# apchenstu/mvsnerf

Hardware: AMD Instinct MI355X
Metric: rendered rays/sec (1024-ray batch, 128 samples) (higher is better)
Workload: dtype f32; 1 GPU; config 2: 3 source views 512x640, 128 depth planes, pad 24 (volume 128x176x208x8), 1024 rays x 128 samples per step, MLP arithmetic fp32, render-only (volume pre-built); weights=mvsnerf-v0 checkpoint, volume=mvsnet-encode, parallelism=ray-sharded x1, no data-path collective

## Files before the change

mvsnerf_amd/csrc/mlp.hip:

```cpp
#include "common.h"
#include "mlp_layout.h"
#include "lds_dma.h"
#include "knobs.h"

using namespace mlp;
typedef float f32x2 __attribute__((ext_vector_type(2)));

struct PackArgs {
    const float* w[11];
    const float* b[11];
    int F;
};

__device__ inline void pack_segment(float* __restrict__ dst, const float* __restrict__ W, int ld, int col_off,
                                    int kmap, int steps, int nb, int F, int tid, int nthreads)
{
    const int total = steps * nb * 64;
    for (int i = tid; i < total; i += nthreads) {
        const int j = i & 3;
        const int lane = (i >> 2) & 63;
        const int rest = i >> 8;
        const int b = rest % nb, t = (rest / nb) * 4 + j;
        const int col = kmap_col(kmap, t, lane >> 5, F);
        const int row = b * 32 + (lane & 31);
        dst[i] = col < 0 ? 0.0f : W[(size_t)row * ld + col_off + col];
    }
}

__global__ __launch_bounds__(256) void mlp_pack_kernel(PackArgs a, float* __restrict__ packed)
{
    const Layout L = layout(a.F);
    const int tid = blockIdx.x * blockDim.x + threadIdx.x, nt = gridDim.x * blockDim.x;
    pack_segment(packed + L.biasw, a.w[6], a.F, 0, K_FEAT, L.fsteps, 4, a.F, tid, nt);
    pack_segment(packed + L.l0, a.w[0], PE_DIM, 0, K_PE, PE_STEPS, 4, a.F, tid, nt);
    pack_segment(packed + L.l1, a.w[1], WIDTH, 0, K_ACT, ACT_STEPS, 4, a.F, tid, nt);
    pack_segment(packed + L.l2, a.w[2], WIDTH, 0, K_ACT, ACT_STEPS, 4, a.F, tid, nt);
// ... 122 lines not shown
    const float v = (q & 1) ? cs : sn;
    return (q & 2) ? -v : v;
}

__device__ __forceinline__ float pe_operand(int t, int half, float px, float py, float pz)
{
    if (t == 0) return half ? py : px;
    if (t == 1) return half ? 0.0f : pz;
    const int j = t - 2, f = j / 3, c = j - 3 * f;
    const float x = (c == 0 ? px : c == 1 ? py : pz) * (float)(1 << f);
    return pe_sin_or_cos(x, half);
}


constexpr int SLAB_FLOATS = 8704;
constexpr int PIPE_LDS_FLOATS = 2 * SLAB_FLOATS + V_TOTAL;

__device__ __forceinline__ void slab_dma(float* __restrict__ dst, const float* __restrict__ src, int n_floats, int wave, int lane)
{
    lds_dma<4>(dst, src, n_floats >> 8, wave, lane);
}
template <int N_FLOATS>
__device__ __forceinline__ void slab_dma_c(float* __restrict__ dst, const float* __restrict__ src, int wave, int lane)
{
    lds_dma_c<4, N_FLOATS / 256>(dst, src, wave, lane);
}

__device__ __forceinline__ void slab_sync()
{
    asm volatile("s_waitcnt vmcnt(0)" ::: "memory");
    __syncthreads();
}

template <bool ALPHA_ONLY, bool SAVE>
__device__ __forceinline__ void mlp_fwd_pipe_tile(
    const unsigned tile, const float* __restrict__ packed, int F, const float* __restrict__ ndc, int ndc_stride,
    const float* __restrict__ feat, int feat_stride, const float* __restrict__ dirs, int dirs_stride,
    int64_t P, int S, float* __restrict__ raw, float* __restrict__ saved, long long* __restrict__ census)
{
    extern __shared__ __attribute__((aligned(16))) float lds[];
    long long t_start = 0, c_start = 0;
    if (census) { t_start = wall_clock64(); c_start = __builtin_amdgcn_s_memtime(); }
    int stamp_i = 4;
    auto stamp = [&]() { if (census && threadIdx.x == 0 && stamp_i < 16) census[tile * 16 + stamp_i] = wall_clock64(); ++stamp_i; };
    float* buf0 = lds;
    float* buf1 = lds + SLAB_FLOATS;
    float* vec = lds + 2 * SLAB_FLOATS;
    constexpr int G = 1;
    const Layout L = layout(F);
    const int tid = threadIdx.x, lane = tid & 63;
    const int wave = __builtin_amdgcn_readfirstlane(tid >> 6);
    const int half = lane >> 5;
    const int64_t p_raw = ((int64_t)tile * 4 + wave) * 32 + (lane & 31);
    const bool live = p_raw < P;
    const int64_t p = live ? p_raw : P - 1;
    float* sv = nullptr;
    if (SAVE) sv = saved + ((int64_t)tile * 4 + wave) * (SLOTS_SAVED * 64) + lane;
    auto save = [&](int slot, float v) { if (SAVE) sv[slot * 64] = v; };
    constexpr int HALF = (int)(ACT_STEPS / 2) * 4 * 64;

    slab_dma(buf0, packed + L.biasw, (int)seg_floats(L.fsteps, 4), wave, lane);
    slab_dma_c<(int)seg_floats(PE_STEPS, 4)>(buf1, packed + L.l0, wave, lane);
    for (int i = tid; i < V_TOTAL; i += 256) vec[i] = packed[L.vec + i];
    const float px = ndc[p * ndc_stride + 0], py = ndc[p * ndc_stride + 1], pz = ndc[p * ndc_stride + 2];
    float fv[MAX_F / 2];
    {
        const float* fp = feat + p * feat_stride + half * (F / 2);
#pragma unroll
        for (int i = 0; i < MAX_F / 2; ++i) fv[i] = i < F / 2 ? fp[i] : 0.0f;
    }
    float bias[64], h[64];
    auto pe = [&](int g, int t) { return pe_operand(t, half, px, py, pz); };
    auto hlo = [&](int g, int t) { return h[t]; };
    auto hhi = [&](int g, int t) { return h[32 + t]; };

    slab_sync();
    stamp();
    {
        f32x16 acc[G][4];
        init_acc<4, G>(acc, vec + V_BIASG + half * 64);
        auto fb = [&](int g, int t) { return fv[t]; };
        switch (L.fsteps) {
            case 4:  gemm_stage<1, 4, G>(buf0, acc, lane, fb); break;
            case 8:  gemm_stage<2, 4, G>(buf0, acc, lane, fb); break;
            case 12: gemm_stage<3, 4, G>(buf0, acc, lane, fb); break;
            case 16: gemm_stage<4, 4, G>(buf0, acc, lane, fb); break;
            default: gemm_stage<5, 4, G>(buf0, acc, lane, fb); break;
        }
#pragma unroll
        for (int q = 0; q < 64; ++q) { bias[q] = acc[0][q >> 4][q & 15]; save(S_BM + q, bias[q]); }
        if (SAVE) {
#pragma unroll
            for (int t = 0; t < 16; ++t) save(S_FV + t, fv[t]);
#pragma unroll
            for (int t = 0; t < PE_STEPS; ++t) save(S_E + t, pe_operand(t, half, px, py, pz));
        }
    }
    stamp();
    slab_sync();
    slab_dma_c<HALF>(buf0, packed + L.l1, wave, lane);
    {
        f32x16 acc[G][4];
        init_acc<4, G>(acc, vec + V_L0 + half * 64);
        gemm_stage<PE_STEPS / 4, 4, G>(buf1, acc, lane, pe);
#pragma unroll
        for (int q = 0; q < 64; q += 2) {
            const f32x2 m2 = f32x2{acc[0][q >> 4][q & 15], acc[0][q >> 4][(q & 15) + 1]} * f32x2{bias[q], bias[q + 1]};
            h[q] = fmaxf(m2[0], 0.0f); h[q + 1] = fmaxf(m2[1], 0.0f);
            save(S_H + q, h[q]); save(S_H + q + 1, h[q + 1]);
// ... 15 lines not shown
            h[q] = fmaxf(m2[0], 0.0f); h[q + 1] = fmaxf(m2[1], 0.0f);
            save(S_H + layer * 64 + q, h[q]); save(S_H + layer * 64 + q + 1, h[q + 1]);
        }
        stamp();
    }
    float sigma;
    {
        f32x16 acc[G][4];
        slab_sync();
        init_acc<4, G>(acc, vec + V_L0 + 128 * 5 + half * 64);
        gemm_stage<PE_STEPS / 4, 4, G>(buf0, acc, lane, pe, [&]() { slab_dma_c<HALF>(buf1, packed + L.l5b, wave, lane); });
        slab_sync();
        gemm_stage<8, 4, G>(buf1, acc, lane, hlo, [&]() { slab_dma_c<HALF>(buf0, packed + L.l5b + HALF, wave, lane); });
        slab_sync();
        gemm_stage<8, 4, G>(buf0, acc, lane, hhi, [&]() { if (!ALPHA_ONLY) slab_dma_c<HALF>(buf1, packed + L.feat, wave, lane); });
#pragma unroll
        for (int q = 0; q < 64; q += 2) {
            const f32x2 m2 = f32x2{acc[0][q >> 4][q & 15], acc[0][q >> 4][(q & 15) + 1]} * f32x2{bias[q], bias[q + 1]};
            h[q] = fmaxf(m2[0], 0.0f); h[q + 1] = fmaxf(m2[1], 0.0f);
            save(S_H + 5 * 64 + q, h[q]); save(S_H + 5 * 64 + q + 1, h[q + 1]);
        }
        const float* wa = vec + V_WA + half * 64;
        float part = 0.0f;
#pragma unroll
        for (int q = 0; q < 64; ++q) part = fmaf(wa[q], h[q], part);
        part += __shfl_xor(part, 32);
        sigma = fmaxf(part + vec[V_BA], 0.0f);
    }
    stamp();
    if (ALPHA_ONLY) {
        if (live && half == 0) raw[p_raw] = sigma;
        return;
    }
    {
        f32x16 acc[G][4];
        slab_sync();
        init_acc<4, G>(acc, vec + V_FEAT + half * 64);
        gemm_stage<8, 4, G>(buf1, acc, lane, hlo, [&]() { slab_dma_c<HALF>(buf0, packed + L.feat + HALF, wave, lane); });
        slab_sync();
        gemm_stage<8, 4, G>(buf0, acc, lane, hhi, [&]() { slab_dma_c<(int)seg_floats(VIEW_STEPS, 2)>(buf1, packed + L.views, wave, lane); });
#pragma unroll
        for (int q = 0; q < 64; ++q) { h[q] = acc[0][q >> 4][q & 15]; save(S_FE + q, h[q]); }
    }
    stamp();
    {
        float d0, d1, d2;
        { const int64_t ray = p / S; d0 = dirs[ray * dirs_stride + 0]; d1 = dirs[ray * dirs_stride + 1]; d2 = dirs[ray * dirs_stride + 2]; }
        f32x16 acc[G][2];
        slab_sync();
        init_acc<2, G>(acc, vec + V_VIEWS + half * 32);
        gemm_stage<VIEW_STEPS / 4, 2, G>(buf1, acc, lane, [&](int g, int t) {
            return t < ACT_STEPS ? h[t < ACT_STEPS ? t : 0] : t == ACT_STEPS ? (half ? d1 : d0) : t == ACT_STEPS + 1 ? (half ? 0.0f : d2) : 0.0f;
        });
        if (SAVE) {
#pragma unroll
            for (int q = 0; q < 32; ++q) save(S_HV + q, fmaxf(acc[0][q >> 4][q & 15], 0.0f));
            save(S_DR + 0, half ? d1 : d0);
            save(S_DR + 1, half ? 0.0f : d2);
        }
        float rgb[3];
#pragma unroll
        for (int c = 0; c < 3; ++c) {
            const float* wr = vec + V_WR + c * 64 + half * 32;
            float part = 0.0f;
#pragma unroll
            for (int q = 0; q < 32; ++q) part = fmaf(wr[q], fmaxf(acc[0][q >> 4][q & 15], 0.0f), part);
            part += __shfl_xor(part, 32);
            const float x = part + vec[V_BR + c];
            rgb[c] = 1.0f / (1.0f + expf(-x));
        }
        if (live && half == 0) *reinterpret_cast<f32x4*>(raw + p_raw * 4) = f32x4{rgb[0], rgb[1], rgb[2], sigma};
    }
    if (census && tid == 0) {
        census[tile * 16 + 0] = t_start;
        census[tile * 16 + 1] = wall_clock64();
        census[tile * 16 + 2] = __builtin_amdgcn_s_getreg((4) | (0 << 6) | (31 << 11));
        census[tile * 16 + 3] = __builtin_amdgcn_s_getreg((20) | (0 << 6) | (31 << 11));
        census[tile * 16 + 13] = __builtin_amdgcn_s_memtime() - c_start;
    }
}

template <bool ALPHA_ONLY, bool SAVE>
__global__ __launch_bounds__(256, 2) void mlp_fwd_pipe_kernel(
    const float* __restrict__ packed, int F, const float* __restrict__ ndc, int ndc_stride,
    const float* __restrict__ feat, int feat_stride, const float* __restrict__ dirs, int dirs_stride,
    int64_t P, int S, float* __restrict__ raw, float* __restrict__ saved, long long* __restrict__ census)
{
    mlp_fwd_pipe_tile<ALPHA_ONLY, SAVE>(blockIdx.x, packed, F, ndc, ndc_stride, feat, feat_stride, dirs, dirs_stride, P, S, raw, saved, census);
}

template <bool ALPHA_ONLY>
__global__ __launch_bounds__(256, 2) void mlp_fwd_pipe_if_kernel(
    const float* __restrict__ packed, int F, const float* __restrict__ ndc, int ndc_stride,
    const float* __restrict__ feat, int feat_stride, const float* __restrict__ dirs, int dirs_stride,
    int64_t P, int S, float* __restrict__ raw, const int* __restrict__ run_if)
{
    if (*run_if == 0) return;
    const unsigned n_tiles = (unsigned)((P + 127) / 128);
    for (unsigned tile = blockIdx.x; tile < n_tiles; tile += gridDim.x) {
        mlp_fwd_pipe_tile<ALPHA_ONLY, false>(tile, packed, F, ndc, ndc_stride, feat, feat_stride, dirs, dirs_stride, P, S, raw, nullptr, nullptr);
        __syncthreads();
    }
}

template <bool AO, bool SAVE>
static int launch_mlp_pipe(const float* packed, int F, const float* ndc, int ndc_stride, const float* feat, int feat_stride,
                           const float* dirs, int dirs_stride, int64_t P, int S, float* raw, hipStream_t st, float* saved = nullptr, long long* census = nullptr,
                           const int* run_if = nullptr)
{
    const size_t lds_bytes = PIPE_LDS_FLOATS * sizeof(float);
    if (run_if) {
        if constexpr (!SAVE) {
            static unsigned long long cap_if = 0;
            if (int rc_ = mvs_raise_lds_cap(reinterpret_cast<const void*>(mlp_fwd_pipe_if_kernel<AO>), (int)lds_bytes, &cap_if)) return rc_;
            const unsigned n_tiles = mvs_cdiv(P, 128);
            mlp_fwd_pipe_if_kernel<AO><<<n_tiles < 512u ? n_tiles : 512u, 256, lds_bytes, st>>>(packed, F, ndc, ndc_stride, feat, feat_stride, dirs, dirs_stride, P, S, raw, run_if);
            MVS_LAUNCH_CHECK();
            return MVSNERF_OK;
        } else {
            return MVSNERF_EINVAL;
        }
    }
    static unsigned long long lds_cap_set = 0;
    if (int rc_ = mvs_raise_lds_cap(reinterpret_cast<const void*>(mlp_fwd_pipe_kernel<AO, SAVE>), (int)lds_bytes, &lds_cap_set)) return rc_;
    mlp_fwd_pipe_kernel<AO, SAVE><<<mvs_cdiv(P, 128), 256, lds_bytes, st>>>(packed, F, ndc, ndc_stride, feat, feat_stride, dirs, dirs_stride, P, S, raw, saved, census);
    MVS_LAUNCH_CHECK();
    return MVSNERF_OK;
}


static int mlp_fwd_checked(const float* packed, int F, const float* ndc, int ndc_stride, const float* feat, int feat_stride,
                           const float* dirs, int dirs_stride, int64_t N, int S, int alpha_only, float* raw, void* stream, long long* census,
                           const int* run_if = nullptr)
{
    if (!packed || !ndc || !feat || !raw || N < 0 || S < 1 || feat_stride < F || ndc_stride < 3) return MVSNERF_EINVAL;
    if (!alpha_only && dirs_stride < 3) return MVSNERF_EINVAL;
    if (!alpha_only && !dirs) return MVSNERF_EINVAL;
    if (F < 2 || F > MAX_F || (F & 1)) return MVSNERF_EUNSUPPORTED;
    if (!mvs_aligned16(packed) || !mvs_aligned16(raw)) return MVSNERF_EALIGN;
    const int64_t P = N * S;
    if (P == 0) return MVSNERF_OK;
    hipStream_t st = (hipStream_t)stream;
    if (alpha_only) return launch_mlp_pipe<true, false>(packed, F, ndc, ndc_stride, feat, feat_stride, dirs, dirs_stride, P, S, raw, st, nullptr, census, run_if);
    return launch_mlp_pipe<false, false>(packed, F, ndc, ndc_stride, feat, feat_stride, dirs, dirs_stride, P, S, raw, st, nullptr, census, run_if);
}

int mvs_mlp_fwd_if(const float* packed, int F, const float* ndc, int ndc_stride, const float* feat, int feat_stride,
                   const float* dirs, int dirs_stride, int64_t N, int S, int alpha_only, float* raw, const int* run_if, void* stream)
{
    return mlp_fwd_checked(packed, F, ndc, ndc_stride, feat, feat_stride, dirs, dirs_stride, N, S, alpha_only, raw, stream, nullptr, run_if);
}

extern "C" int mvsnerf_mlp_fwd(const float* packed, int F, const float* ndc, int ndc_stride, const float* feat, int feat_stride,
                               const float* dirs, int dirs_stride, int64_t N, int S, int alpha_only, float* raw, void* stream)
{
    return mlp_fwd_checked(packed, F, ndc, ndc_stride, feat, feat_stride, dirs, dirs_stride, N, S, alpha_only, raw, stream, nullptr);
}

extern "C" int mvsnerf_mlp_fwd_census(const float* packed, int F, const float* ndc, int ndc_stride, const float* feat, int feat_stride,
                                      const float* dirs, int dirs_stride, int64_t N, int S, int alpha_only, float* raw, long long* census, void* stream)
{
    if (!census) return MVSNERF_EINVAL;
// ... 15 lines not shown
```

mvsnerf_amd/csrc/raymarch.hip:

```cpp
#include "common.h"

extern "C" int mvsnerf_abi_version(void) { return 12; }

int mvs_mlp_f16x3_fwd(const void* packed_h, const float* packed_f32, int F, const float* ndc, int ndc_stride, const float* feat, int feat_stride,
                      const float* dirs, int dirs_stride, int64_t P, int S, int alpha_only, float* raw, hipStream_t st, int* guard);
int mvs_mlp_fwd_if(const float* packed, int F, const float* ndc, int ndc_stride, const float* feat, int feat_stride,
                   const float* dirs, int dirs_stride, int64_t N, int S, int alpha_only, float* raw, const int* run_if, void* stream);
int mvs_composite_fwd(const float* raw, const float* z, int64_t N, int S, int white_bkgd, float* rgb_map, float* disp, float* acc, float* weights,
                      float* depth, float* alpha, int* guard, void* stream);
int mvs_guard_consume(int* guard, hipStream_t st);

static int mlp_guarded_pair(const void* packed_h, const float* packed_f32, int F, const float* ndc, int ndc_stride, const float* feat, int feat_stride,
                            const float* dirs, int dirs_stride, int64_t N, int S, int alpha_only, float* raw, int* guard, void* stream)
{
    if (!packed_h || !packed_f32 || !ndc || !feat || !raw || !guard || N < 0 || S < 1 || feat_stride < F || ndc_stride < 3) return MVSNERF_EINVAL;
    if (!alpha_only && (!dirs || dirs_stride < 3)) return MVSNERF_EINVAL;
    if (F < 2 || F > 40 || (F & 1)) return MVSNERF_EUNSUPPORTED;
    if (!mvs_aligned16(packed_h) || !mvs_aligned16(packed_f32) || !mvs_aligned16(raw)) return MVSNERF_EALIGN;
    if (N * S == 0) return MVSNERF_OK;
    if (int rc = mvs_mlp_f16x3_fwd(packed_h, packed_f32, F, ndc, ndc_stride, feat, feat_stride, dirs, dirs_stride, N * S, S, alpha_only, raw, (hipStream_t)stream, guard)) return rc;
    return mvs_mlp_fwd_if(packed_f32, F, ndc, ndc_stride, feat, feat_stride, dirs, dirs_stride, N, S, alpha_only, raw, guard, stream);
}

extern "C" int mvsnerf_mlp_fwd_guarded(const void* packed_fp16, const float* packed_f32, int F, const float* ndc, int ndc_stride,
                                       const float* feat, int feat_stride, const float* dirs, int dirs_stride,
                                       int64_t N, int S, int alpha_only, float* raw, int* guard, void* stream)
{
    if (int rc = mlp_guarded_pair(packed_fp16, packed_f32, F, ndc, ndc_stride, feat, feat_stride, dirs, dirs_stride, N, S, alpha_only, raw, guard, stream)) return rc;
    if (N * S == 0) return MVSNERF_OK;
    return mvs_guard_consume(guard, (hipStream_t)stream);
}

extern "C" int mvsnerf_raymarch_fwd(const mvsnerf_raymarch_args* a, void* stream)
{
    if (!a) return MVSNERF_EINVAL;
    if (!a->vol || !a->imgs || !a->w2c || !a->K || !a->packed_mlp || !a->rays_pts || !a->rays_ndc || !a->z_vals ||
        !a->rays_dir || !a->dirs_tmp || !a->input_feat || !a->raw)
        return MVSNERF_EINVAL;
    if (a->N < 0 || a->S < 1 || a->V < 1) return MVSNERF_EINVAL;
    const int F = 8 + 4 * a->V;
    const int64_t P = a->N * a->S;
    int rc;
    if (a->imgs_nhwc4) {
        if ((rc = mvsnerf_gather_fwd(a->vol, a->D, a->H, a->W, a->imgs_nhwc4, a->V, a->IH, a->IW, a->w2c, a->K, a->rays_pts, a->rays_ndc,
                                     a->N, a->S, a->rays_dir, a->input_feat, F, a->dirs_tmp, a->vol_layout, stream))) return rc;
    } else {
        if ((rc = mvsnerf_dir_feature_fwd(a->rays_dir, a->w2c, a->N, 1, a->dirs_tmp, stream))) return rc;
        if ((rc = mvsnerf_volume_sample_fwd(a->vol, a->D, a->H, a->W, 8, a->rays_ndc, P, a->input_feat, F, a->vol_layout, stream))) return rc;
        if ((rc = mvsnerf_color_sample_fwd(a->imgs, a->V, a->IH, a->IW, a->w2c, a->K, a->rays_pts, P, 1, a->input_feat + 8, F, stream))) return rc;
    }
    const bool guarded = a->guard && a->packed_mlp_split && a->n_split == MVSNERF_SPLIT_FP16;
    if (a->guard && !guarded) return MVSNERF_EINVAL;
    if (guarded)
        rc = mlp_guarded_pair(a->packed_mlp_split, a->packed_mlp, F, a->rays_ndc, 3, a->input_feat, F, a->dirs_tmp, 3, a->N, a->S, 0, a->raw, a->guard, stream);
    else if (a->packed_mlp_split)
        rc = mvsnerf_mlp_fwd_split(a->packed_mlp_split, a->packed_mlp, F, a->n_split, a->rays_ndc, 3, a->input_feat, F, a->dirs_tmp, 3, a->N, a->S, 0, a->raw, stream);
    else if (a->packed_mlp_bf16)
        rc = mvsnerf_mlp_fwd_bf16(a->packed_mlp_bf16, a->packed_mlp, F, a->rays_ndc, 3, a->input_feat, F, a->dirs_tmp, 3, a->N, a->S, 0, a->raw, stream);
    else
        rc = mvsnerf_mlp_fwd(a->packed_mlp, F, a->rays_ndc, 3, a->input_feat, F, a->dirs_tmp, 3, a->N, a->S, 0, a->raw, stream);
    if (rc) return rc;
    return mvs_composite_fwd(a->raw, a->z_vals, a->N, a->S, a->white_bkgd, a->rgb_map, a->disp, a->acc, a->weights, a->depth, a->alpha,
                             guarded && P > 0 ? a->guard : nullptr, stream);
}

extern "C" int mvsnerf_raymarch_fwd_batched(const mvsnerf_raymarch_args* a, int K, void* stream)
{
    if (!a || K < 0) return MVSNERF_EINVAL;
    for (int k = 0; k < K; ++k)
        if (int rc = mvsnerf_raymarch_fwd(a + k, stream)) return rc;
    return MVSNERF_OK;
}

static size_t render_ws_floats(int64_t B, int S, int V)
{
// ... 5 lines not shown
extern "C" size_t mvsnerf_render_workspace_floats(int batch_rays, int S, int V)
{
    if (batch_rays < 1 || S < 1 || V < 1) return 0;
    return render_ws_floats(batch_rays, S, V);
}

extern "C" int mvsnerf_render_pixels_fwd(const mvsnerf_render_args* a, void* stream)
{
    if (!a) return MVSNERF_EINVAL;
    if (a->n_pixels == 0) return MVSNERF_OK;
    if (!a->vol || !a->imgs_nhwc4 || !a->w2c || !a->K || !a->packed_mlp || !a->K_tgt || !a->c2w_tgt || !a->K_ref || !a->w2c_ref ||
        !a->near_far_tgt || !a->near_far_ref || !a->workspace || !a->rgb)
        return MVSNERF_EINVAL;
    if (a->n_pixels < 0 || a->first_pixel < 0 || a->S < 1 || a->V < 1 || a->batch_rays < 1 || a->W_img < 2 || a->H_img < 2) return MVSNERF_EINVAL;
    if (a->first_pixel + a->n_pixels > (int64_t)a->W_img * a->H_img) return MVSNERF_EINVAL;
    if (a->workspace_floats < render_ws_floats(a->batch_rays, a->S, a->V)) return MVSNERF_EINVAL;
    const int F = 8 + 4 * a->V, S = a->S;
    const bool guarded = a->guard && a->packed_mlp_split && a->n_split == MVSNERF_SPLIT_FP16;
    if (a->guard && !guarded) return MVSNERF_EINVAL;
    const int64_t B = a->batch_rays, P = B * S;
    auto r4 = [](int64_t n) { return (n + 3) & ~(int64_t)3; };
    float* pts = a->workspace;
    float* ndc = pts + r4(3 * P);
    float* z = ndc + r4(3 * P);
    float* feat = z + r4(P);
    float* raw = feat + r4((int64_t)F * P);
    float* rdir = raw + r4(4 * P);
    float* dirs = rdir + r4(3 * B);
    int rc;
    for (int64_t off = 0; off < a->n_pixels; off += B) {
        const int64_t n = a->n_pixels - off < B ? a->n_pixels - off : B;
        if ((rc = mvsnerf_raygen_fwd(nullptr, nullptr, a->first_pixel + off, a->W_img, a->H_img, a->W_ref, a->H_ref, a->K_tgt, a->c2w_tgt, a->K_ref, a->w2c_ref,
                                     a->near_far_tgt, a->near_far_ref, a->pad, a->lindisp, nullptr, n, S, pts, rdir, ndc, z, nullptr, stream))) return rc;
        if ((rc = mvsnerf_gather_fwd(a->vol, a->D, a->H, a->W, a->imgs_nhwc4, a->V, a->IH, a->IW, a->w2c, a->K, pts, ndc, n, S, rdir,
                                     feat, F, dirs, a->vol_layout, stream))) return rc;
        if (guarded)
            rc = mlp_guarded_pair(a->packed_mlp_split, a->packed_mlp, F, ndc, 3, feat, F, dirs, 3, n, S, 0, raw, a->guard, stream);
        else if (a->packed_mlp_split)
            rc = mvsnerf_mlp_fwd_split(a->packed_mlp_split, a->packed_mlp, F, a->n_split, ndc, 3, feat, F, dirs, 3, n, S, 0, raw, stream);
        else if (a->packed_mlp_bf16)
            rc = mvsnerf_mlp_fwd_bf16(a->packed_mlp_bf16, a->packed_mlp, F, ndc, 3, feat, F, dirs, 3, n, S, 0, raw, stream);
        else
            rc = mvsnerf_mlp_fwd(a->packed_mlp, F, ndc, 3, feat, F, dirs, 3, n, S, 0, raw, stream);
        if (rc) return rc;
        if ((rc = mvs_composite_fwd(raw, z, n, S, a->white_bkgd, a->rgb + off * 3, a->disp ? a->disp + off : nullptr,
                                    a->acc ? a->acc + off : nullptr, nullptr, a->depth ? a->depth + off : nullptr, nullptr,
                                    guarded ? a->guard : nullptr, stream))) return rc;
    }
    return MVSNERF_OK;
}

extern "C" int mvsnerf_raymarch_train_fwd(const mvsnerf_raymarch_train_args* a, void* stream)
{
    if (!a) return MVSNERF_EINVAL;
    if (!a->vol || !a->w2c || !a->packed_mlp || !a->rays_ndc || !a->z_vals || !a->rays_dir || !a->dirs_tmp || !a->input_feat || !a->raw || !a->saved)
        return MVSNERF_EINVAL;
    if (a->N < 0 || a->S < 1 || a->V < 1 || (a->bf16 && !a->packed_mlp_bf16)) return MVSNERF_EINVAL;
    const int F = 8 + 4 * a->V;
    const int64_t P = a->N * a->S;
    int rc;
    if (a->C == F && a->C != 8) {
        if ((rc = mvsnerf_dir_feature_fwd(a->rays_dir, a->w2c, a->N, 1, a->dirs_tmp, stream))) return rc;
        if ((rc = mvsnerf_volume_sample_fwd(a->vol, a->D, a->H, a->W, a->C, a->rays_ndc, P, a->input_feat, F, a->vol_layout, stream))) return rc;
    } else if (a->C == 8) {
        if (!a->imgs_nhwc4 || !a->K || !a->rays_pts) return MVSNERF_EINVAL;
        if ((rc = mvsnerf_gather_fwd(a->vol, a->D, a->H, a->W, a->imgs_nhwc4, a->V, a->IH, a->IW, a->w2c, a->K, a->rays_pts, a->rays_ndc,
// ... 31 lines not shown
```

mvsnerf_amd/csrc/sample.hip:

```cpp
#include "common.h"
#include "sample_dev.h"
#include <type_traits>

template <int SPQ, bool SMALL>
__global__ __launch_bounds__(256) void volume_sample_c8_kernel(
    const float* __restrict__ vol, int D, int H, int W,
    const float* __restrict__ ndc, int64_t P, float* __restrict__ out, int out_stride)
{
#pragma clang fp contract(off)
    const int64_t tid = (int64_t)blockIdx.x * blockDim.x + threadIdx.x;
    const int q = (int)(tid & 3);
    const int xc = q >> 1, ch = (q & 1) * 4;
    const int64_t p0 = (tid >> 2) * SPQ;
    f32x4 acc[SPQ];
#pragma unroll
    for (int j = 0; j < SPQ; ++j) {
        const int64_t p = p0 + j;
        const int64_t pc = p < P ? p : (P - 1);
        typedef float f32x3 __attribute__((ext_vector_type(3)));
        const f32x3 nd = *reinterpret_cast<const f32x3*>(ndc + pc * 3);
        const float gx = nd[0] * 2.0f - 1.0f;
        const float gy = nd[1] * 2.0f - 1.0f;
        const float gz = nd[2] * 2.0f - 1.0f;
        const float ix = ((gx + 1.0f) / 2.0f) * (float)(W - 1);
// ... 210 lines not shown
    f32x4 vv[4];
    float vw[4];
    ZfastTaps zt;
    if constexpr (ZFAST) {
        zt = zfast_taps<SMALL>(a.vol, D, H, W, a.ndc[p * 3 + 0], a.ndc[p * 3 + 1], a.ndc[p * 3 + 2], q);
    } else {
        const float gx = a.ndc[p * 3 + 0] * 2.0f - 1.0f;
        const float gy = a.ndc[p * 3 + 1] * 2.0f - 1.0f;
        const float gz = a.ndc[p * 3 + 2] * 2.0f - 1.0f;
        const float ix = ((gx + 1.0f) / 2.0f) * (float)(W - 1);
        const float iy = ((gy + 1.0f) / 2.0f) * (float)(H - 1);
        const float iz = ((gz + 1.0f) / 2.0f) * (float)(D - 1);
        const float fx = floorf(ix), fy = floorf(iy), fz = floorf(iz);
        const float wx = xc ? (ix - fx) : ((fx + 1.0f) - ix);
        const float cxf = fx + (float)xc;
        const bool x_in = (cxf >= 0.0f) && (cxf <= (float)(W - 1));
#pragma unroll
        for (int k = 0; k < 4; ++k) {
            const int zc = k >> 1, yc = k & 1;
            const float cyf = fy + (float)yc, czf = fz + (float)zc;
            const bool in = x_in && (cyf >= 0.0f) && (cyf <= (float)(H - 1)) && (czf >= 0.0f) && (czf <= (float)(D - 1));
            vw[k] = (wx * (yc ? (iy - fy) : ((fy + 1.0f) - iy))) * (zc ? (iz - fz) : ((fz + 1.0f) - iz));
            const float* src = in ? a.vol + vox_off8<SMALL>((int)czf, (int)cyf, (int)cxf, H, W) + ch : reinterpret_cast<const float*>(&g_zero_tap);
            vv[k] = ldg16(src);
        }
    }
    typedef float f32x3 __attribute__((ext_vector_type(3)));
    const f32x3 pp = *reinterpret_cast<const f32x3*>(a.pts + p * 3);
    const float px = pp[0], py = pp[1], pz = pp[2];
    float* frow = a.feat + p * (idx_t)a.feat_stride;
    for (int v = q; v < a.V; v += 4) {
        const int IW = a.IW, IH = a.IH;
        const ColorTap t = color_project(px, py, pz, a.w2c + v * 16, a.Kmat + v * 9, IW, IH);
        const float* pl = a.img + (SMALL ? (int64_t)((__umul24(v * IH + t.y0, IW) + t.x0) << 2) : (((int64_t)v * IH + t.y0) * IW + t.x0) * 4);
        const float* zt = reinterpret_cast<const float*>(&g_zero_tap);
        const f32x4 t_nw = ldg16(pl);
        const f32x4 t_ne = ldg16(t.x1in ? pl + 4 : zt);
        const f32x4 t_sw = ldg16(t.y1in ? pl + (int64_t)IW * 4 : zt);
        const f32x4 t_se = ldg16((t.x1in && t.y1in) ? pl + (int64_t)IW * 4 + 4 : zt);
        f32x4 o;
#pragma unroll
        for (int c = 0; c < 3; ++c) o[c] = color_blend(t, t_nw[c], t_ne[c], t_sw[c], t_se[c]);
        o[3] = color_mask(t);
        if (live) *reinterpret_cast<f32x4*>(frow + 8 + 4 * v) = o;
    }
    if constexpr (ZFAST) {
        const f32x4 acc = zfast_fold_y0_lane(zt);
        if (live && q < 2) *reinterpret_cast<f32x4*>(frow + q * 4) = acc;
    } else {
        const f32x4 acc = trilinear_fold_x0_lane(vv, vw);
        if (live && xc == 0) *reinterpret_cast<f32x4*>(frow + ch) = acc;
    }
    if (q == 3 && a.dirs_out && p_raw < a.N) dir_feature_of(a.rays_dir + p_raw * 3, a.w2c, 1, a.dirs_out + p_raw * 3);
}

extern "C" int mvsnerf_gather_fwd(const float* vol, int D, int H, int W, const float* imgs_nhwc4, int V, int IH, int IW,
                                  const float* w2c, const float* K, const float* pts, const float* ndc, int64_t N, int S,
                                  const float* rays_dir, float* feat, int feat_stride, float* dirs_out, int vol_layout, void* stream)
{
    if (vol_layout != MVSNERF_VOL_DHWC && vol_layout != MVSNERF_VOL_HWDC) return MVSNERF_EINVAL;
    if (!vol || !imgs_nhwc4 || !w2c || !K || !pts || !ndc || !feat || D < 1 || H < 1 || W < 1 || V < 1 || IH < 2 || IW < 2 || N < 0 || S < 1)
        return MVSNERF_EINVAL;
    if (dirs_out && !rays_dir) return MVSNERF_EINVAL;
    if (feat_stride < 8 + 4 * V) return MVSNERF_EINVAL;
    if ((feat_stride & 3) || !mvs_aligned16(feat) || !mvs_aligned16(vol) || !mvs_aligned16(imgs_nhwc4)) return MVSNERF_EALIGN;
    if (N == 0) return MVSNERF_OK;
    const int64_t P = N * S;
    const GatherArgs a{vol, D, H, W, imgs_nhwc4, V, IH, IW, w2c, K, pts, ndc, P, N, rays_dir, feat, feat_stride, dirs_out};
    const bool small = (int64_t)D * H < (1 << 24) && W < (1 << 24) && (int64_t)H * W < (1 << 24) && D < (1 << 24) && (int64_t)D * H * W * 8 < ((int64_t)1 << 31) &&
                       (int64_t)V * IH < (1 << 24) && IW < (1 << 24) && (int64_t)V * IH * IW * 4 < ((int64_t)1 << 31) &&
                       P * (int64_t)(feat_stride > 3 ? feat_stride : 3) < ((int64_t)1 << 31);
    const unsigned grid = mvs_cdiv(P * 4, 256);
    hipStream_t st = (hipStream_t)stream;
    if (vol_layout == MVSNERF_VOL_HWDC) {
        if (small) gather_fused_kernel<true, true><<<grid, 256, 0, st>>>(a);
        else gather_fused_kernel<false, true><<<grid, 256, 0, st>>>(a);
    } else {
        if (small) gather_fused_kernel<true, false><<<grid, 256, 0, st>>>(a);
        else gather_fused_kernel<false, false><<<grid, 256, 0, st>>>(a);
    }
    MVS_LAUNCH_CHECK();
    return MVSNERF_OK;
}

__global__ __launch_bounds__(256) void ncdhw_to_ndhwc_kernel(const float* __restrict__ src, float* __restrict__ dst, int C, int64_t n_vox)
{
    const int64_t i = (int64_t)blockIdx.x * blockDim.x + threadIdx.x;
    if (i >= n_vox) return;
    for (int c = 0; c < C; ++c) dst[i * C + c] = src[(int64_t)c * n_vox + i];
}
__global__ __launch_bounds__(256) void ndhwc_to_ncdhw_kernel(const float* __restrict__ src, float* __restrict__ dst, int C, int64_t n_vox)
{
    const int64_t i = (int64_t)blockIdx.x * blockDim.x + threadIdx.x;
    if (i >= n_vox) return;
    for (int c = 0; c < C; ++c) dst[(int64_t)c * n_vox + i] = src[i * C + c];
}

extern "C" int mvsnerf_ncdhw_to_ndhwc(const float* src, float* dst, int C, int D, int H, int W, void* stream)
{
    if (!src || !dst || C < 1 || D < 1 || H < 1 || W < 1) return MVSNERF_EINVAL;
    const int64_t n = (int64_t)D * H * W;
    ncdhw_to_ndhwc_kernel<<<mvs_cdiv(n, 256), 256, 0, (hipStream_t)stream>>>(src, dst, C, n);
    MVS_LAUNCH_CHECK();
    return MVSNERF_OK;
// ... 356 lines not shown
```

mvsnerf_amd/csrc/sample_dev.h:

```cpp
#pragma once
#include "common.h"

static __device__ const f32x4 g_zero_tap = {0.0f, 0.0f, 0.0f, 0.0f};

__device__ __forceinline__ f32x4 ldg16(const float* p)
{
    typedef const f32x4 __attribute__((address_space(1))) * gptr;
    return *(gptr)p;
}

template <bool SMALL>
__device__ __forceinline__ int64_t vox_off8(int z, int y, int x, int H, int W)
{
    if constexpr (SMALL) return (int64_t)((__umul24(__umul24(z, H) + y, W) + x) << 3);
    else return (((int64_t)z * H + y) * W + x) << 3;
}

__device__ __forceinline__ float quad_swap2(float v)
{
    return __int_as_float(__builtin_amdgcn_update_dpp(0, __float_as_int(v), 0x4e, 0xf, 0xf, false));
}

struct ColorTap { float gx, gy, wnw, wne, wsw, wse; int x0, y0; bool x1in, y1in; };

// ... 4 lines not shown
    const float cx = fmaf(z, M[2],  fmaf(y, M[1], x * M[0]))  + M[3];
    const float cy = fmaf(z, M[6],  fmaf(y, M[5], x * M[4]))  + M[7];
    const float cz = fmaf(z, M[10], fmaf(y, M[9], x * M[8]))  + M[11];
    const float qx = fmaf(cz, K[2], fmaf(cy, K[1], cx * K[0]));
    const float qy = fmaf(cz, K[5], fmaf(cy, K[4], cx * K[3]));
    const float qz = fmaf(cz, K[8], fmaf(cy, K[7], cx * K[6]));
    t.gx = ((qx / qz + 0.0f) / (float)(W - 1)) * 2.0f - 1.0f;
    t.gy = ((qy / qz + 0.0f) / (float)(H - 1)) * 2.0f - 1.0f;
    float ix = ((t.gx + 1.0f) / 2.0f) * (float)(W - 1);
    float iy = ((t.gy + 1.0f) / 2.0f) * (float)(H - 1);
    ix = fminf(fmaxf(ix, 0.0f), (float)(W - 1));
    iy = fminf(fmaxf(iy, 0.0f), (float)(H - 1));
    if (!(ix == ix)) ix = 0.0f;
    if (!(iy == iy)) iy = 0.0f;
    const float fx = floorf(ix), fy = floorf(iy);
    t.x0 = (int)fx; t.y0 = (int)fy;
    const float wx1 = ix - fx, wx0 = (fx + 1.0f) - ix, wy1 = iy - fy, wy0 = (fy + 1.0f) - iy;
    t.x1in = t.x0 + 1 <= W - 1; t.y1in = t.y0 + 1 <= H - 1;
    t.wnw = wx0 * wy0; t.wne = wx1 * wy0; t.wsw = wx0 * wy1; t.wse = wx1 * wy1;
    return t;
}

__device__ __forceinline__ float color_blend(const ColorTap& t, float nw, float ne, float sw, float se)
{
#pragma clang fp contract(off)
    float acc = nw * t.wnw;
    if (t.x1in) acc = fmaf(ne, t.wne, acc);
    if (t.y1in) acc = fmaf(sw, t.wsw, acc);
    if (t.x1in && t.y1in) acc = fmaf(se, t.wse, acc);
    return acc;
}

__device__ __forceinline__ float color_mask(const ColorTap& t) { return (t.gx > -1.0f && t.gx < 1.0f && t.gy > -1.0f && t.gy < 1.0f) ? 1.0f : 0.0f; }

__device__ __forceinline__ void dir_feature_of(const float* __restrict__ d3, const float* __restrict__ R, int normalize, float* __restrict__ o3)
{
#pragma clang fp contract(off)
    const float dx = d3[0], dy = d3[1], dz = d3[2];
    const float nrm = normalize ? sqrtf(fmaf(dz, dz, fmaf(dy, dy, dx * dx))) : 1.0f;
    const float ux = dx / nrm, uy = dy / nrm, uz = dz / nrm;
    if (R) {
        o3[0] = fmaf(uz, R[2],  fmaf(uy, R[1], ux * R[0]));
        o3[1] = fmaf(uz, R[6],  fmaf(uy, R[5], ux * R[4]));
        o3[2] = fmaf(uz, R[10], fmaf(uy, R[9], ux * R[8]));
    } else {
        o3[0] = ux; o3[1] = uy; o3[2] = uz;
    }
}


__device__ __forceinline__ f32x4 trilinear_fold_x0_lane(const f32x4 (&v)[4], const float (&w)[4])
{
#pragma clang fp contract(off)
    f32x4 acc = {0.0f, 0.0f, 0.0f, 0.0f};
#pragma unroll
    for (int k = 0; k < 4; ++k) {
        const f32x4 own = v[k] * w[k];
        f32x4 other;
#pragma unroll
        for (int c = 0; c < 4; ++c) other[c] = quad_swap2(own[c]);
        acc = acc + own;
        acc = acc + other;
    }
    return acc;
}

// ... 2 lines not shown
{
    if constexpr (SMALL) return (int64_t)((__umul24(__umul24(y, W) + x, D) + z) << 3);
    else return ((((int64_t)y * W + x) * D + z) << 3);
}

struct ZfastTaps { f32x4 v[4]; float w[4]; };

template <bool SMALL>
__device__ __forceinline__ ZfastTaps zfast_taps(const float* __restrict__ vol, int D, int H, int W, float nx, float ny, float nz, int q)
{
#pragma clang fp contract(off)
    ZfastTaps t;
    const float gx = nx * 2.0f - 1.0f, gy = ny * 2.0f - 1.0f, gz = nz * 2.0f - 1.0f;
    const float ix = ((gx + 1.0f) / 2.0f) * (float)(W - 1);
    const float iy = ((gy + 1.0f) / 2.0f) * (float)(H - 1);
    const float iz = ((gz + 1.0f) / 2.0f) * (float)(D - 1);
    const float fx = floorf(ix), fy = floorf(iy), fz = floorf(iz);
    const int yc = q >> 1, ch = (q & 1) * 4;
    const float wy = yc ? (iy - fy) : ((fy + 1.0f) - iy);
    const float cyf = fy + (float)yc;
    const bool y_in = (cyf >= 0.0f) && (cyf <= (float)(H - 1));
    const float* zt = reinterpret_cast<const float*>(&g_zero_tap);
#pragma unroll
    for (int k = 0; k < 4; ++k) {
        const int zc = k >> 1, xc = k & 1;
        const float cxf = fx + (float)xc, czf = fz + (float)zc;
        const bool in = y_in && (cxf >= 0.0f) && (cxf <= (float)(W - 1)) && (czf >= 0.0f) && (czf <= (float)(D - 1));
        t.w[k] = ((xc ? (ix - fx) : ((fx + 1.0f) - ix)) * wy) * (zc ? (iz - fz) : ((fz + 1.0f) - iz));
        t.v[k] = ldg16(in ? vol + vox_off8_zfast<SMALL>((int)czf, (int)cyf, (int)cxf, D, W) + ch : zt);
    }
    return t;
}

__device__ __forceinline__ f32x4 zfast_fold_y0_lane(const ZfastTaps& t)
{
#pragma clang fp contract(off)
    f32x4 acc = {0.0f, 0.0f, 0.0f, 0.0f};
#pragma unroll
    for (int z = 0; z < 2; ++z) {
        const f32x4 a = t.v[2 * z] * t.w[2 * z], b = t.v[2 * z + 1] * t.w[2 * z + 1];
        f32x4 pa, pb;
#pragma unroll
        for (int c = 0; c < 4; ++c) { pa[c] = quad_swap2(a[c]); pb[c] = quad_swap2(b[c]); }
        acc = acc + a;
        acc = acc + b;
        acc = acc + pa;
        acc = acc + pb;
    }
    return acc;
}
```

Measured before the change: 4.033 million rays/s.

## Fuse gather, MLP and compositing into one raymarch kernel per tile

Adds a fused kernel that performs the volume and source-image lookups for a 128-point tile directly into LDS, runs the MLP on those staged features, computes the view direction feature in-kernel, and composites whole rays inside the tile when rays fit evenly. This removes separate gather and composite launches and the global round trip of features between them. Feature rows are still written out to global for compatibility, the fused path only triggers when unguarded and fp32 MLP, and LDS staging may delay the first weight DMA when space is tight.

```diff
diff --git a/mvsnerf_amd/csrc/mlp.hip b/mvsnerf_amd/csrc/mlp.hip
--- a/mvsnerf_amd/csrc/mlp.hip
+++ b/mvsnerf_amd/csrc/mlp.hip
@@ -2,6 +2,8 @@
 #include "mlp_layout.h"
 #include "lds_dma.h"
 #include "knobs.h"
+#include "sample_dev.h"
+#include "composite_wave.h"
 
 using namespace mlp;
 typedef float f32x2 __attribute__((ext_vector_type(2)));
@@ -190,11 +192,83 @@
     __syncthreads();
 }
 
-template <bool ALPHA_ONLY, bool SAVE>
+struct RaymarchTileArgs {
+    const float* vol; int D, H, W;
+    const float* img; int V, IH, IW;
+    const float* w2c; const float* Kmat;
+    const float* pts; const float* rays_dir;
+    float* feat; float* dirs_out;
+    const float* z; int64_t N; int rays_per_tile;
+    CompositeOut o;
+};
+
+__device__ __forceinline__ void tile_lookups(const unsigned tile, const RaymarchTileArgs& a, const float* __restrict__ ndc, int64_t P, int F,
+                                             float* __restrict__ stage)
+{
+#pragma clang fp contract(off)
+    const int tid = threadIdx.x, q = tid & 3;
+    int r[2];
+    bool live[2];
+    unsigned p[2];
+    ZfastTaps zt[2];
+    ColorTap ct[2][2];
+    f32x3 tap[2][2][4];
+    f32x3 nn[2], pp[2];
+#pragma unroll
+    for (int ps = 0; ps < 2; ++ps) {
+        r[ps] = ps * 64 + (tid >> 2);
+        const int64_t p_raw = (int64_t)tile * 128 + r[ps];
+        live[ps] = p_raw < P;
+        p[ps] = (unsigned)(live[ps] ? p_raw : P - 1);
+        nn[ps] = f32x3{ndc[p[ps] * 3 + 0], ndc[p[ps] * 3 + 1], ndc[p[ps] * 3 + 2]};
+        pp[ps] = *reinterpret_cast<const f32x3*>(a.pts + p[ps] * 3);
+    }
+    const bool two = a.V > 4;
+    const int vk[2] = {q < a.V ? q : a.V - 1, q + 4 < a.V ? q + 4 : a.V - 1};
+    float Mv[2][12], Kv[2][9];
+#pragma unroll
+    for (int k = 0; k < 2; ++k)
+        if (k == 0 || two) {
+#pragma unroll
+            for (int i = 0; i < 12; ++i) Mv[k][i] = a.w2c[vk[k] * 16 + i];
+#pragma unroll
+            for (int i = 0; i < 9; ++i) Kv[k][i] = a.Kmat[vk[k] * 9 + i];
+        }
+#pragma unroll
+    for (int ps = 0; ps < 2; ++ps) zt[ps] = zfast_taps<true>(a.vol, a.D, a.H, a.W, nn[ps][0], nn[ps][1], nn[ps][2], q);
+#pragma unroll
+    for (int ps = 0; ps < 2; ++ps)
+#pragma unroll
+        for (int k = 0; k < 2; ++k)
+            if (k == 0 || two) {
+                ct[ps][k] = color_project(pp[ps][0], pp[ps][1], pp[ps][2], Mv[k], Kv[k], a.IW, a.IH);
+                color_taps_nhwc4<true, f32x3>(a.img, vk[k], a.IH, a.IW, ct[ps][k], tap[ps][k]);
+            }
+#pragma unroll
+    for (int ps = 0; ps < 2; ++ps) {
+        float* srow = stage + r[ps] * F;
+#pragma unroll
+        for (int k = 0; k < 2; ++k)
+            if ((k == 0 || two) && q + 4 * k < a.V) *reinterpret_cast<f32x4*>(srow + 8 + 16 * k + 4 * q) = color_row(ct[ps][k], tap[ps][k]);
+        const f32x4 acc = zfast_fold_y0_lane(zt[ps]);
+        if (q < 2) *reinterpret_cast<f32x4*>(srow + q * 4) = acc;
+    }
+}
+
+__device__ __forceinline__ void tile_rows_out(const unsigned tile, float* __restrict__ feat, const float* __restrict__ stage, int64_t P, int F)
+{
+    const int64_t row0 = (int64_t)tile * 128;
+    const int n4 = (int)(P - row0 < 128 ? P - row0 : 128) * (F / 4);
+    f32x4* dst = reinterpret_cast<f32x4*>(feat + row0 * F);
+    const f32x4* src = reinterpret_cast<const f32x4*>(stage);
+    for (int i = threadIdx.x; i < n4; i += 256) dst[i] = src[i];
+}
+
+template <bool ALPHA_ONLY, bool SAVE, bool FUSED = false, int NR = 0>
 __device__ __forceinline__ void mlp_fwd_pipe_tile(
     const unsigned tile, const float* __restrict__ packed, int F, const float* __restrict__ ndc, int ndc_stride,
     const float* __restrict__ feat, int feat_stride, const float* __restrict__ dirs, int dirs_stride,
-    int64_t P, int S, float* __restrict__ raw, float* __restrict__ saved, long long* __restrict__ census)
+    int64_t P, int S, float* __restrict__ raw, float* __restrict__ saved, long long* __restrict__ census, const RaymarchTileArgs* fa = nullptr)
 {
     extern __shared__ __attribute__((aligned(16))) float lds[];
     long long t_start = 0, c_start = 0;
@@ -217,12 +291,37 @@
     auto save = [&](int slot, float v) { if (SAVE) sv[slot * 64] = v; };
     constexpr int HALF = (int)(ACT_STEPS / 2) * 4 * 64;
 
+    constexpr int VEC_PER_THREAD = (V_TOTAL + 255) / 256;
+    float vec_pre[VEC_PER_THREAD];
+    if constexpr (FUSED) {
+#pragma unroll
+        for (int k = 0; k < VEC_PER_THREAD; ++k) vec_pre[k] = tid + 256 * k < V_TOTAL ? packed[L.vec + tid + 256 * k] : 0.0f;
+    }
     slab_dma(buf0, packed + L.biasw, (int)seg_floats(L.fsteps, 4), wave, lane);
-    slab_dma_c<(int)seg_floats(PE_STEPS, 4)>(buf1, packed + L.l0, wave, lane);
-    for (int i = tid; i < V_TOTAL; i += 256) vec[i] = packed[L.vec + i];
+    const bool l0_first = !FUSED || seg_floats(L.fsteps, 4) + 128 * (size_t)F <= SLAB_FLOATS;
+    float* stage = l0_first ? buf0 + seg_floats(L.fsteps, 4) : buf1;
+    if (l0_first) slab_dma_c<(int)seg_floats(PE_STEPS, 4)>(buf1, packed + L.l0, wave, lane);
+    if constexpr (FUSED) {
+        tile_lookups(tile, *fa, ndc, P, F, stage);
+#pragma unroll
+        for (int k = 0; k < VEC_PER_THREAD; ++k)
+            if (tid + 256 * k < V_TOTAL) vec[tid + 256 * k] = vec_pre[k];
+    } else {
+        for (int i = tid; i < V_TOTAL; i += 256) vec[i] = packed[L.vec + i];
+    }
     const float px = ndc[p * ndc_stride + 0], py = ndc[p * ndc_stride + 1], pz = ndc[p * ndc_stride + 2];
     float fv[MAX_F / 2];
-    {
+    if constexpr (FUSED) {
+        slab_sync();
+        const float* fp = stage + (wave * 32 + (lane & 31)) * F + half * (F / 2);
+#pragma unroll
+        for (int i = 0; i < MAX_F / 2; ++i) fv[i] = i < F / 2 ? fp[i] : 0.0f;
+        tile_rows_out(tile, fa->feat, stage, P, F);
+        if (!l0_first) {
+            __syncthreads();
+            slab_dma_c<(int)seg_floats(PE_STEPS, 4)>(buf1, packed + L.l0, wave, lane);
+        }
+    } else {
         const float* fp = feat + p * feat_stride + half * (F / 2);
 #pragma unroll
         for (int i = 0; i < MAX_F / 2; ++i) fv[i] = i < F / 2 ? fp[i] : 0.0f;
@@ -232,7 +331,7 @@
     auto hlo = [&](int g, int t) { return h[t]; };
     auto hhi = [&](int g, int t) { return h[32 + t]; };
 
-    slab_sync();
+    if constexpr (!FUSED) slab_sync();
     stamp();
     {
         f32x16 acc[G][4];
@@ -314,6 +413,15 @@
         if (live && half == 0) raw[p_raw] = sigma;
         return;
     }
+    float rdir[3] = {0.0f, 0.0f, 0.0f}, rot[11];
+    int64_t ray_of_p = 0;
+    if constexpr (FUSED) {
+        ray_of_p = p / S;
+#pragma unroll
+        for (int c = 0; c < 3; ++c) rdir[c] = fa->rays_dir[ray_of_p * 3 + c];
+#pragma unroll
+        for (int i = 0; i < 11; ++i) rot[i] = fa->w2c[i];
+    }
     {
         f32x16 acc[G][4];
         slab_sync();
@@ -326,8 +434,19 @@
     }
     stamp();
     {
+        float z_pre = 0.0f;
+        if constexpr (FUSED && NR > 0)
+            if (tid < 128 && (int64_t)tile * 128 + tid < P) z_pre = fa->z[(int64_t)tile * 128 + tid];
         float d0, d1, d2;
-        { const int64_t ray = p / S; d0 = dirs[ray * dirs_stride + 0]; d1 = dirs[ray * dirs_stride + 1]; d2 = dirs[ray * dirs_stride + 2]; }
+        if constexpr (FUSED) {
+            const int64_t ray = ray_of_p;
+            float d[3];
+            dir_feature_of(rdir, rot, 1, d);
+            d0 = d[0]; d1 = d[1]; d2 = d[2];
+            if (live && half == 0 && p_raw == ray * S) { fa->dirs_out[ray * 3 + 0] = d0; fa->dirs_out[ray * 3 + 1] = d1; fa->dirs_out[ray * 3 + 2] = d2; }
+        } else {
+            const int64_t ray = p / S; d0 = dirs[ray * dirs_stride + 0]; d1 = dirs[ray * dirs_stride + 1]; d2 = dirs[ray * dirs_stride + 2];
+        }
         f32x16 acc[G][2];
         slab_sync();
         init_acc<2, G>(acc, vec + V_VIEWS + half * 32);
@@ -352,6 +471,24 @@
             rgb[c] = 1.0f / (1.0f + expf(-x));
         }
         if (live && half == 0) *reinterpret_cast<f32x4*>(raw + p_raw * 4) = f32x4{rgb[0], rgb[1], rgb[2], sigma};
+        if constexpr (FUSED && NR > 0) {
+            if (half == 0) reinterpret_cast<f32x4*>(buf0)[wave * 32 + (lane & 31)] = f32x4{rgb[0], rgb[1], rgb[2], sigma};
+            float* zs = buf0 + 4 * 128;
+            if (tid < 128) zs[tid] = z_pre;
+            __syncthreads();
+            const f32x4* rs = reinterpret_cast<const f32x4*>(buf0);
+            for (int rl = wave; rl < fa->rays_per_tile; rl += 4) {
+                const int64_t ray = (int64_t)tile * fa->rays_per_tile + rl;
+                if (ray >= fa->N) break;
+                f32x4 rv[NR];
+#pragma unroll
+                for (int i = 0; i < NR; ++i) {
+                    const int s = lane * NR + i;
+                    rv[i] = s < S ? rs[rl * S + s] : f32x4{0, 0, 0, 0};
+                }
+                composite_wave<NR>(rv, zs + rl * S, ray, S, lane, fa->o);
+            }
+        }
     }
     if (census && tid == 0) {
         census[tile * 16 + 0] = t_start;
@@ -410,6 +547,48 @@
     return MVSNERF_OK;
 }
 
+template <int NR>
+__global__ __launch_bounds__(256, 2) void raymarch_fused_kernel(const float* __restrict__ packed, int F, const float* __restrict__ ndc, int64_t P, int S,
+                                                                float* __restrict__ raw, RaymarchTileArgs fa)
+{
+    mlp_fwd_pipe_tile<false, false, true, NR>(blockIdx.x, packed, F, ndc, 3, nullptr, F, nullptr, 3, P, S, raw, nullptr, nullptr, &fa);
+}
+
+int mvs_composite_fwd(const float* raw, const float* z, int64_t N, int S, int white_bkgd, float* rgb_map, float* disp, float* acc, float* weights,
+                      float* depth, float* alpha, int* guard, void* stream);
+int mvs_raymarch_fused_fwd(const float* vol, int D, int H, int W, int vol_layout, const float* imgs_nhwc4, int V, int IH, int IW, const float* w2c,
+                           const float* K, const float* packed, const float* pts, const float* ndc, const float* z, int64_t N, int S,
+                           const float* rays_dir, float* feat, float* dirs_out, float* raw, int white_bkgd, float* rgb_map, float* disp, float* acc,
+                           float* weights, float* depth, float* alpha, void* stream, bool* taken)
+{
+    *taken = false;
+    const int F = 8 + 4 * V;
+    if (vol_layout != MVSNERF_VOL_HWDC || !vol || !imgs_nhwc4 || !w2c || !K || !packed || !pts || !ndc || !z || !rays_dir || !feat || !dirs_out || !raw) return MVSNERF_OK;
+    if (D < 1 || H < 1 || W < 1 || V < 1 || F > MAX_F || IH < 2 || IW < 2 || N < 1 || S < 1) return MVSNERF_OK;
+    if (!mvs_aligned16(feat) || !mvs_aligned16(vol) || !mvs_aligned16(imgs_nhwc4) || !mvs_aligned16(packed) || !mvs_aligned16(raw)) return MVSNERF_OK;
+    const int64_t P = N * S;
+    if (!gather_fits_32bit(D, H, W, V, IH, IW, P, F)) return MVSNERF_OK;
+    *taken = true;
+    const RaymarchTileArgs fa{vol, D, H, W, imgs_nhwc4, V, IH, IW, w2c, K, pts, rays_dir, feat, dirs_out, z, N, 128 % S == 0 ? 128 / S : 0,
+                              CompositeOut{rgb_map, disp, acc, weights, depth, alpha, white_bkgd, nullptr}};
+    hipStream_t st = (hipStream_t)stream;
+    const size_t lds_bytes = PIPE_LDS_FLOATS * sizeof(float);
+    const unsigned grid = mvs_cdiv(P, 128);
+    static unsigned long long cap[3] = {0, 0, 0};
+#define MVS_FUSED(NR_)                                                                                                                 \
+    do {                                                                                                                               \
+        if (int rc_ = mvs_raise_lds_cap(reinterpret_cast<const void*>(raymarch_fused_kernel<NR_>), (int)lds_bytes, &cap[NR_])) return rc_; \
+        raymarch_fused_kernel<NR_><<<grid, 256, lds_bytes, st>>>(packed, F, ndc, P, S, raw, fa);                                     \
+    } while (0)
+    if (fa.rays_per_tile == 0) MVS_FUSED(0);
+    else if (S <= 64) MVS_FUSED(1);
+    else MVS_FUSED(2);
+#undef MVS_FUSED
+    MVS_LAUNCH_CHECK();
+    if (fa.rays_per_tile == 0)
+        return mvs_composite_fwd(raw, z, N, S, white_bkgd, rgb_map, disp, acc, weights, depth, alpha, nullptr, stream);
+    return MVSNERF_OK;
+}
 
 static int mlp_fwd_checked(const float* packed, int F, const float* ndc, int ndc_stride, const float* feat, int feat_stride,
                            const float* dirs, int dirs_stride, int64_t N, int S, int alpha_only, float* raw, void* stream, long long* census,
diff --git a/mvsnerf_amd/csrc/raymarch.hip b/mvsnerf_amd/csrc/raymarch.hip
--- a/mvsnerf_amd/csrc/raymarch.hip
+++ b/mvsnerf_amd/csrc/raymarch.hip
@@ -9,6 +9,10 @@
 int mvs_composite_fwd(const float* raw, const float* z, int64_t N, int S, int white_bkgd, float* rgb_map, float* disp, float* acc, float* weights,
                       float* depth, float* alpha, int* guard, void* stream);
 int mvs_guard_consume(int* guard, hipStream_t st);
+int mvs_raymarch_fused_fwd(const float* vol, int D, int H, int W, int vol_layout, const float* imgs_nhwc4, int V, int IH, int IW, const float* w2c,
+                           const float* K, const float* packed, const float* pts, const float* ndc, const float* z, int64_t N, int S,
+                           const float* rays_dir, float* feat, float* dirs_out, float* raw, int white_bkgd, float* rgb_map, float* disp, float* acc,
+                           float* weights, float* depth, float* alpha, void* stream, bool* taken);
 
 static int mlp_guarded_pair(const void* packed_h, const float* packed_f32, int F, const float* ndc, int ndc_stride, const float* feat, int feat_stride,
                             const float* dirs, int dirs_stride, int64_t N, int S, int alpha_only, float* raw, int* guard, void* stream)
@@ -41,6 +45,12 @@
     const int F = 8 + 4 * a->V;
     const int64_t P = a->N * a->S;
     int rc;
+    if (a->imgs_nhwc4 && !a->packed_mlp_split && !a->packed_mlp_bf16 && !a->guard) {
+        bool taken;
+        if ((rc = mvs_raymarch_fused_fwd(a->vol, a->D, a->H, a->W, a->vol_layout, a->imgs_nhwc4, a->V, a->IH, a->IW, a->w2c, a->K, a->packed_mlp,
+                                         a->rays_pts, a->rays_ndc, a->z_vals, a->N, a->S, a->rays_dir, a->input_feat, a->dirs_tmp, a->raw, a->white_bkgd,
+                                         a->rgb_map, a->disp, a->acc, a->weights, a->depth, a->alpha, stream, &taken)) || taken) return rc;
+    }
     if (a->imgs_nhwc4) {
         if ((rc = mvsnerf_gather_fwd(a->vol, a->D, a->H, a->W, a->imgs_nhwc4, a->V, a->IH, a->IW, a->w2c, a->K, a->rays_pts, a->rays_ndc,
                                      a->N, a->S, a->rays_dir, a->input_feat, F, a->dirs_tmp, a->vol_layout, stream))) return rc;
@@ -112,6 +122,13 @@
         const int64_t n = a->n_pixels - off < B ? a->n_pixels - off : B;
         if ((rc = mvsnerf_raygen_fwd(nullptr, nullptr, a->first_pixel + off, a->W_img, a->H_img, a->W_ref, a->H_ref, a->K_tgt, a->c2w_tgt, a->K_ref, a->w2c_ref,
                                      a->near_far_tgt, a->near_far_ref, a->pad, a->lindisp, nullptr, n, S, pts, rdir, ndc, z, nullptr, stream))) return rc;
+        if (!guarded && !a->packed_mlp_split && !a->packed_mlp_bf16) {
+            bool taken;
+            if ((rc = mvs_raymarch_fused_fwd(a->vol, a->D, a->H, a->W, a->vol_layout, a->imgs_nhwc4, a->V, a->IH, a->IW, a->w2c, a->K, a->packed_mlp, pts,
+                                             ndc, z, n, S, rdir, feat, dirs, raw, a->white_bkgd, a->rgb + off * 3, a->disp ? a->disp + off : nullptr,
+                                             a->acc ? a->acc + off : nullptr, nullptr, a->depth ? a->depth + off : nullptr, nullptr, stream, &taken))) return rc;
+            if (taken) continue;
+        }
         if ((rc = mvsnerf_gather_fwd(a->vol, a->D, a->H, a->W, a->imgs_nhwc4, a->V, a->IH, a->IW, a->w2c, a->K, pts, ndc, n, S, rdir,
                                      feat, F, dirs, a->vol_layout, stream))) return rc;
         if (guarded)
diff --git a/mvsnerf_amd/csrc/sample.hip b/mvsnerf_amd/csrc/sample.hip
--- a/mvsnerf_amd/csrc/sample.hip
+++ b/mvsnerf_amd/csrc/sample.hip
@@ -266,17 +266,9 @@
     for (int v = q; v < a.V; v += 4) {
         const int IW = a.IW, IH = a.IH;
         const ColorTap t = color_project(px, py, pz, a.w2c + v * 16, a.Kmat + v * 9, IW, IH);
-        const float* pl = a.img + (SMALL ? (int64_t)((__umul24(v * IH + t.y0, IW) + t.x0) << 2) : (((int64_t)v * IH + t.y0) * IW + t.x0) * 4);
-        const float* zt = reinterpret_cast<const float*>(&g_zero_tap);
-        const f32x4 t_nw = ldg16(pl);
-        const f32x4 t_ne = ldg16(t.x1in ? pl + 4 : zt);
-        const f32x4 t_sw = ldg16(t.y1in ? pl + (int64_t)IW * 4 : zt);
-        const f32x4 t_se = ldg16((t.x1in && t.y1in) ? pl + (int64_t)IW * 4 + 4 : zt);
-        f32x4 o;
-#pragma unroll
-        for (int c = 0; c < 3; ++c) o[c] = color_blend(t, t_nw[c], t_ne[c], t_sw[c], t_se[c]);
-        o[3] = color_mask(t);
-        if (live) *reinterpret_cast<f32x4*>(frow + 8 + 4 * v) = o;
+        f32x4 tap[4];
+        color_taps_nhwc4<SMALL>(a.img, v, IH, IW, t, tap);
+        if (live) *reinterpret_cast<f32x4*>(frow + 8 + 4 * v) = color_row(t, tap);
     }
     if constexpr (ZFAST) {
         const f32x4 acc = zfast_fold_y0_lane(zt);
@@ -301,9 +293,7 @@
     if (N == 0) return MVSNERF_OK;
     const int64_t P = N * S;
     const GatherArgs a{vol, D, H, W, imgs_nhwc4, V, IH, IW, w2c, K, pts, ndc, P, N, rays_dir, feat, feat_stride, dirs_out};
-    const bool small = (int64_t)D * H < (1 << 24) && W < (1 << 24) && (int64_t)H * W < (1 << 24) && D < (1 << 24) && (int64_t)D * H * W * 8 < ((int64_t)1 << 31) &&
-                       (int64_t)V * IH < (1 << 24) && IW < (1 << 24) && (int64_t)V * IH * IW * 4 < ((int64_t)1 << 31) &&
-                       P * (int64_t)(feat_stride > 3 ? feat_stride : 3) < ((int64_t)1 << 31);
+    const bool small = gather_fits_32bit(D, H, W, V, IH, IW, P, feat_stride);
     const unsigned grid = mvs_cdiv(P * 4, 256);
     hipStream_t st = (hipStream_t)stream;
     if (vol_layout == MVSNERF_VOL_HWDC) {
diff --git a/mvsnerf_amd/csrc/sample_dev.h b/mvsnerf_amd/csrc/sample_dev.h
--- a/mvsnerf_amd/csrc/sample_dev.h
+++ b/mvsnerf_amd/csrc/sample_dev.h
@@ -60,6 +60,35 @@
 }
 
 __device__ __forceinline__ float color_mask(const ColorTap& t) { return (t.gx > -1.0f && t.gx < 1.0f && t.gy > -1.0f && t.gy < 1.0f) ? 1.0f : 0.0f; }
+
+typedef float f32x3 __attribute__((ext_vector_type(3)));
+template <typename PIX>
+__device__ __forceinline__ PIX ldg_pix(const float* p)
+{
+    typedef const PIX __attribute__((address_space(1))) * gptr;
+    return *(gptr)p;
+}
+
+template <bool SMALL, typename PIX = f32x4>
+__device__ __forceinline__ void color_taps_nhwc4(const float* __restrict__ img, int v, int IH, int IW, const ColorTap& t, PIX (&tap)[4])
+{
+    const float* pl = img + (SMALL ? (int64_t)((__umul24(v * IH + t.y0, IW) + t.x0) << 2) : (((int64_t)v * IH + t.y0) * IW + t.x0) * 4);
+    const float* zt = reinterpret_cast<const float*>(&g_zero_tap);
+    tap[0] = ldg_pix<PIX>(pl);
+    tap[1] = ldg_pix<PIX>(t.x1in ? pl + 4 : zt);
+    tap[2] = ldg_pix<PIX>(t.y1in ? pl + (int64_t)IW * 4 : zt);
+    tap[3] = ldg_pix<PIX>((t.x1in && t.y1in) ? pl + (int64_t)IW * 4 + 4 : zt);
+}
+
+template <typename PIX>
+__device__ __forceinline__ f32x4 color_row(const ColorTap& t, const PIX (&tap)[4])
+{
+    f32x4 o;
+#pragma unroll
+    for (int c = 0; c < 3; ++c) o[c] = color_blend(t, tap[0][c], tap[1][c], tap[2][c], tap[3][c]);
+    o[3] = color_mask(t);
+    return o;
+}
 
 __device__ __forceinline__ void dir_feature_of(const float* __restrict__ d3, const float* __restrict__ R, int normalize, float* __restrict__ o3)
 {
@@ -128,6 +157,13 @@
     return t;
 }
 
+inline bool gather_fits_32bit(int D, int H, int W, int V, int IH, int IW, int64_t P, int feat_stride)
+{
+    return (int64_t)D * H < (1 << 24) && W < (1 << 24) && (int64_t)H * W < (1 << 24) && D < (1 << 24) && (int64_t)D * H * W * 8 < ((int64_t)1 << 31) &&
+           (int64_t)V * IH < (1 << 24) && IW < (1 << 24) && (int64_t)V * IH * IW * 4 < ((int64_t)1 << 31) &&
+           P * (int64_t)(feat_stride > 3 ? feat_stride : 3) < ((int64_t)1 << 31);
+}
+
 __device__ __forceinline__ f32x4 zfast_fold_y0_lane(const ZfastTaps& t)
 {
 #pragma clang fp contract(off)
```

Measured after the change: 4.134 million rays/s (median of 6 runs). +2.5%, better.
